# Orbiter-Finance/Plonky2-lib

Hardware: AMD Instinct MI355X
Metric: proofs/sec for secp256k1 ECDSA-verify circuit; Goldilocks NTT GB/s vs HBM peak (higher is better)
Workload: dtype u64 (Goldilocks, 64-bit modular integer)

## Files before the change

plonky2-lib_amd/csrc/merkle.hip:

```cpp
#include "merkle.h"
#include "keccak.h"
#include "poseidon.h"

namespace glp {
using namespace glf;

constexpr size_t MERKLE_COOP_MAX_PARENTS = 8192;

size_t merkle_num_digests(size_t nleaves, int cap_height) {
    size_t t = 0, w = nleaves, cap = (size_t)1 << cap_height;
    for (;;) { t += w; if (w <= cap) break; w >>= 1; }
    return t;
}
size_t merkle_cap_offset(size_t nleaves, int cap_height) {
    return merkle_num_digests(nleaves, cap_height) - ((size_t)1 << cap_height);
}

__device__ __forceinline__ void store_digest(u64 *dst, const u64 s[12]) {
    ulonglong2 a, b;
    a.x = s[0]; a.y = s[1]; b.x = s[2]; b.y = s[3];
    reinterpret_cast<ulonglong2 *>(dst)[0] = a;
    reinterpret_cast<ulonglong2 *>(dst)[1] = b;
}

__global__ __launch_bounds__(256, 4) void k_leaf_hash_lde(const u64 *__restrict__ lde, u64 *__restrict__ digests,
                                                       u32 ncols, int lg, int rate_bits, size_t lde_stride, size_t dig_stride) {
    lde += (size_t)blockIdx.y * lde_stride; digests += (size_t)blockIdx.y * dig_stride;
    const size_t N = (size_t)1 << (lg + rate_bits);
    const size_t pos = (size_t)blockIdx.x * 256 + threadIdx.x;
    if (pos >= N) return;
    const u32 r = (u32)(pos >> lg), q = (u32)(pos & (((size_t)1 << lg) - 1));
    const size_t leaf = ((size_t)bitrev32(r, rate_bits) << lg) | bitrev32(q, lg);
    u64 s[12];
#pragma unroll
    for (int i = 0; i < 12; i++) s[i] = 0;
    const u64 *p = lde + pos;
    if (ncols <= 4) {
        for (u32 c = 0; c < ncols; c++) s[c] = p[(size_t)c * N];
    } else {
        u64 nx[8];
#pragma unroll
        for (int i = 0; i < 8; i++) nx[i] = i < (int)ncols ? p[(size_t)i * N] : 0;
        for (u32 c = 0; c < ncols; c += 8) {
#pragma unroll
            for (int i = 0; i < 8; i++)
                if (c + i < ncols) s[i] = nx[i];
            if (c + 8 < ncols) {
#pragma unroll
                for (int i = 0; i < 8; i++)
                    if (c + 8 + i < ncols) nx[i] = p[(size_t)(c + 8 + i) * N];
            }
            pos::permute(s);
        }
    }
    store_digest(digests + 4 * leaf, s);
}

__global__ __launch_bounds__(256) void k_leaf_hash_lde_coop(const u64 *__restrict__ lde, u64 *__restrict__ digests,
                                                            u32 ncols, int lg, int rate_bits, size_t lde_stride, size_t dig_stride) {
    lde += (size_t)blockIdx.y * lde_stride; digests += (size_t)blockIdx.y * dig_stride;
    const size_t N = (size_t)1 << (lg + rate_bits);
    const int tid = threadIdx.x, l = tid & 15, lane = tid & 63, group_base = lane & ~15;
    const size_t pos = (size_t)blockIdx.x * 16 + (tid >> 4);
    const bool live = pos < N;
    const size_t p = live ? pos : 0;
    const u32 r = (u32)(p >> lg), q = (u32)(p & (((size_t)1 << lg) - 1));
    const size_t leaf = ((size_t)bitrev32(r, rate_bits) << lg) | bitrev32(q, lg);
    u64 x = 0;
    if (ncols <= 4) {
        if (live && l < 4) digests[4 * leaf + l] = (u32)l < ncols ? lde[(size_t)l * N + p] : 0;
        return;
    }
    for (u32 c = 0; c < ncols; c += 8) {
        if (l < 8 && c + l < ncols) x = lde[(size_t)(c + l) * N + p];
        x = pos::permute_coop(x, l, group_base);
    }
    if (live && l < 4) digests[4 * leaf + l] = x;
}

__global__ __launch_bounds__(256) void k_leaf_hash_lde_quad(const u64 *__restrict__ lde, u64 *__restrict__ digests,
                                                            u32 ncols, int lg, int rate_bits, size_t lde_stride, size_t dig_stride) {
    lde += (size_t)blockIdx.y * lde_stride; digests += (size_t)blockIdx.y * dig_stride;
    const size_t N = (size_t)1 << (lg + rate_bits);
    const int tid = threadIdx.x, q = tid & 3;
    const size_t pos = (size_t)blockIdx.x * 64 + (tid >> 2);
    const bool live = pos < N;
    const size_t p = live ? pos : 0;
    const u32 r = (u32)(p >> lg), qq = (u32)(p & (((size_t)1 << lg) - 1));
    const size_t leaf = ((size_t)bitrev32(r, rate_bits) << lg) | bitrev32(qq, lg);
    if (ncols <= 4) {
        if (live) digests[4 * leaf + q] = (u32)q < ncols ? lde[(size_t)q * N + p] : 0;
        return;
    }
    u64 x[3] = {0, 0, 0};
    for (u32 c = 0; c < ncols; c += 8) {
#pragma unroll
        for (int s = 0; s < 3; s++) {
            const u32 e = 3 * q + s;
            if (e < 8 && c + e < ncols) x[s] = lde[(size_t)(c + e) * N + p];
        }
        pos::permute_quad(x, q);
    }
    if (live) {
        if (q == 0) { digests[4 * leaf] = x[0]; digests[4 * leaf + 1] = x[1]; digests[4 * leaf + 2] = x[2]; }
        if (q == 1) digests[4 * leaf + 3] = x[0];
    }
}

__global__ __launch_bounds__(256, 4) void k_leaf_hash_rows(const u64 *__restrict__ rows, u64 *__restrict__ digests,
                                                        size_t nleaves, u32 leaf_len) {
    const size_t j = (size_t)blockIdx.x * 256 + threadIdx.x;
    if (j >= nleaves) return;
    u64 s[12];
#pragma unroll
    for (int i = 0; i < 12; i++) s[i] = 0;
    const u64 *p = rows + j * leaf_len;
    if (leaf_len <= 4) {
        for (u32 c = 0; c < leaf_len; c++) s[c] = p[c];
    } else {
        u32 c = 0;
        for (; c + 8 <= leaf_len; c += 8) {
#pragma unroll
            for (int i = 0; i < 8; i++) s[i] = p[c + i];
            pos::permute(s);
        }
        if (c < leaf_len) {
#pragma unroll
            for (int i = 0; i < 8; i++)
                if (c + i < leaf_len) s[i] = p[c + i];
            pos::permute(s);
        }
    }
    store_digest(digests + 4 * j, s);
}

__global__ __launch_bounds__(256) void k_merkle_level(const u64 *__restrict__ in, u64 *__restrict__ out, size_t m, size_t dig_stride) {
    in += (size_t)blockIdx.y * dig_stride; out += (size_t)blockIdx.y * dig_stride;
    const size_t i = (size_t)blockIdx.x * 256 + threadIdx.x;
    if (i >= m) return;
    const ulonglong2 *src = reinterpret_cast<const ulonglong2 *>(in + 8 * i);
    ulonglong2 a = src[0], b = src[1], c2 = src[2], d = src[3];
    u64 s[12] = {a.x, a.y, b.x, b.y, c2.x, c2.y, d.x, d.y, 0, 0, 0, 0};
    pos::permute(s);
    store_digest(out + 4 * i, s);
}

__global__ __launch_bounds__(256) void k_merkle_level_coop(const u64 *__restrict__ in, u64 *__restrict__ out, size_t m, size_t dig_stride) {
    in += (size_t)blockIdx.y * dig_stride; out += (size_t)blockIdx.y * dig_stride;
    const int tid = threadIdx.x, l = tid & 15, lane = tid & 63, group_base = lane & ~15;
    const size_t i = (size_t)blockIdx.x * 16 + (tid >> 4);
    const bool live = i < m;
    u64 x = (live && l < 8) ? in[8 * i + l] : 0;
    x = pos::permute_coop(x, l, group_base);
    if (live && l < 4) out[4 * i + l] = x;
}

__global__ __launch_bounds__(256) void k_merkle_level_quad(const u64 *__restrict__ in, u64 *__restrict__ out, size_t m, size_t dig_stride) {
    in += (size_t)blockIdx.y * dig_stride; out += (size_t)blockIdx.y * dig_stride;
    const int tid = threadIdx.x, q = tid & 3;
    const size_t i0 = (size_t)blockIdx.x * 64 + (tid >> 2);
    const bool live = i0 < m;
    const size_t i = live ? i0 : 0;
    u64 x[3];
#pragma unroll
    for (int s = 0; s < 3; s++) x[s] = 3 * q + s < 8 ? in[8 * i + 3 * q + s] : 0;
    pos::permute_quad(x, q);
    if (live) {
        if (q == 0) { out[4 * i] = x[0]; out[4 * i + 1] = x[1]; out[4 * i + 2] = x[2]; }
        if (q == 1) out[4 * i + 3] = x[0];
    }
}

__global__ void k_permute_states(u64 *states, size_t count) {
    const size_t i = (size_t)blockIdx.x * blockDim.x + threadIdx.x;
    if (i >= count) return;
    u64 s[12];
#pragma unroll
    for (int k = 0; k < 12; k++) s[k] = states[12 * i + k];
    pos::permute(s);
#pragma unroll
    for (int k = 0; k < 12; k++) states[12 * i + k] = s[k];
}

__global__ __launch_bounds__(256) void k_leaf_hash_lde_keccak(const u64 *__restrict__ lde, u64 *__restrict__ digests, u32 ncols, int lg,
                                                              int rate_bits, size_t lde_stride, size_t dig_stride) {
    lde += (size_t)blockIdx.y * lde_stride; digests += (size_t)blockIdx.y * dig_stride;
    const size_t N = (size_t)1 << (lg + rate_bits);
    const size_t pos = (size_t)blockIdx.x * 256 + threadIdx.x;
    if (pos >= N) return;
    const u32 r = (u32)(pos >> lg), q = (u32)(pos & (((size_t)1 << lg) - 1));
    const size_t leaf = ((size_t)bitrev32(r, rate_bits) << lg) | bitrev32(q, lg);
    const u64 *p = lde + pos;
    u64 d[4] = {0, 0, 0, 0};
    if (ncols <= 3) {
        for (u32 c = 0; c < ncols; c++) d[c] = p[(size_t)c * N];
    } else {
        kec::Sponge s;
        kec::sponge_init(s);
        u32 c = 0;
        for (; c + kec::RATE_LANES <= ncols; c += kec::RATE_LANES) {
#pragma unroll
            for (int i = 0; i < kec::RATE_LANES; i++) s.a[i] ^= p[(size_t)(c + i) * N];
            kec::f1600(s.a);
        }
#pragma unroll
        for (int i = 0; i < kec::RATE_LANES; i++) if (c + i < ncols) s.a[i] ^= p[(size_t)(c + i) * N];
        s.fill = (int)(ncols - c);
        kec::sponge_finish(s);
        kec::sponge_digest25(s, d);
    }
    store_digest(digests + 4 * leaf, d);
}
__global__ __launch_bounds__(256) void k_merkle_level_keccak(const u64 *__restrict__ in, u64 *__restrict__ out, size_t m, size_t dig_stride) {
    in += (size_t)blockIdx.y * dig_stride; out += (size_t)blockIdx.y * dig_stride;
    const size_t i = (size_t)blockIdx.x * 256 + threadIdx.x;
    if (i >= m) return;
    const ulonglong2 *src = reinterpret_cast<const ulonglong2 *>(in + 8 * i);
    const ulonglong2 a = src[0], b = src[1], c2 = src[2], e = src[3];
    const u64 l[4] = {a.x, a.y, b.x, b.y}, r[4] = {c2.x, c2.y, e.x, e.y};
    u64 d[4];
    kec::two_to_one(l, r, d);
    store_digest(out + 4 * i, d);
}

static int build_levels(glp_ctx *c, u64 *dev_digests, size_t nleaves, int cap_height, u32 K = 1, size_t dig_stride = 0, int hasher = 0) {
    size_t w = nleaves, cap = (size_t)1 << cap_height;
    u64 *lvl = dev_digests;
    while (w > cap) {
        u64 *nxt = lvl + 4 * w;
        size_t m = w >> 1;
        if (hasher == GLP_HASH_KECCAK25)
            hipLaunchKernelGGL(k_merkle_level_keccak, dim3((unsigned)((m + 255) / 256), K), dim3(256), 0, c->stream, lvl, nxt, m, dig_stride);
        else if (m * K <= MERKLE_COOP_MAX_PARENTS)
            hipLaunchKernelGGL(k_merkle_level_coop, dim3((unsigned)((m + 15) / 16), K), dim3(256), 0, c->stream, lvl, nxt, m, dig_stride);
        else if (m * K <= c->merkle_quad_max)
            hipLaunchKernelGGL(k_merkle_level_quad, dim3((unsigned)((m + 63) / 64), K), dim3(256), 0, c->stream, lvl, nxt, m, dig_stride);
        else
            hipLaunchKernelGGL(k_merkle_level, dim3((unsigned)((m + 255) / 256), K), dim3(256), 0, c->stream, lvl, nxt, m, dig_stride);
        GLP_HIP(hipGetLastError());
        lvl = nxt; w = m;
    }
    return GLP_OK;
}

int merkle_levels(glp_ctx *c, u64 *dev_digests, size_t nleaves, int cap_height, u32 K, size_t dig_stride, int hasher) {
    return build_levels(c, dev_digests, nleaves, cap_height, K, dig_stride, hasher);
}

int merkle_from_lde(glp_ctx *c, const u64 *dev_lde, u32 ncols, int lg, int rate_bits, int cap_height, u64 *dev_digests, u32 K,
                    size_t lde_stride, size_t dig_stride, int hasher) {
    const size_t N = (size_t)1 << (lg + rate_bits);
    if (cap_height < 0 || ((size_t)1 << cap_height) > N)
        return set_error(GLP_ERR_ARG, "cap_height=%d should be at most log2(leaves)=%d", cap_height, lg + rate_bits);
    GLP_REQUIRE(K >= 1 && K <= 65535, "batch of %u trees outside 1..65535", K);
    {
        StageScope st(c, "merkle_leaves", (double)N * K * (8.0 * ncols + 32.0));
        if (hasher == GLP_HASH_KECCAK25)
            hipLaunchKernelGGL(k_leaf_hash_lde_keccak, dim3((unsigned)((N + 255) / 256), K), dim3(256), 0, c->stream, dev_lde, dev_digests,
                               ncols, lg, rate_bits, lde_stride, dig_stride);
        else if (N * K <= c->merkle_coop_max)
            hipLaunchKernelGGL(k_leaf_hash_lde_coop, dim3((unsigned)((N + 15) / 16), K), dim3(256), 0, c->stream, dev_lde, dev_digests,
                               ncols, lg, rate_bits, lde_stride, dig_stride);
        else if (N * K <= c->merkle_quad_max)
            hipLaunchKernelGGL(k_leaf_hash_lde_quad, dim3((unsigned)((N + 63) / 64), K), dim3(256), 0, c->stream, dev_lde, dev_digests,
                               ncols, lg, rate_bits, lde_stride, dig_stride);
        else
            hipLaunchKernelGGL(k_leaf_hash_lde, dim3((unsigned)((N + 255) / 256), K), dim3(256), 0, c->stream, dev_lde, dev_digests,
                               ncols, lg, rate_bits, lde_stride, dig_stride);
        GLP_HIP(hipGetLastError());
    }
    StageScope st(c, "merkle_levels", (double)N * K * 32.0 * 1.5);
    return build_levels(c, dev_digests, N, cap_height, K, dig_stride, hasher);
}

int merkle_from_rows(glp_ctx *c, const u64 *dev_rows, size_t nleaves, u32 leaf_len, int cap_height, u64 *dev_digests) {
    if (cap_height < 0 || ((size_t)1 << cap_height) > nleaves)
        return set_error(GLP_ERR_ARG, "cap_height=%d should be at most log2(leaves)", cap_height);
    hipLaunchKernelGGL(k_leaf_hash_rows, dim3((unsigned)((nleaves + 255) / 256)), dim3(256), 0, c->stream, dev_rows,
                       dev_digests, nleaves, leaf_len);
    GLP_HIP(hipGetLastError());
    return build_levels(c, dev_digests, nleaves, cap_height);
}

__global__ void k_gather_lde_rows(const u64 *__restrict__ lde, u32 ncols, int lg, int rate_bits,
                                  const u64 *__restrict__ leaf_idx, u32 count, u64 *__restrict__ out, size_t out_stride,
                                  size_t lde_bstride, size_t out_bstride) {
    lde += (size_t)blockIdx.y * lde_bstride; leaf_idx += (size_t)blockIdx.y * count; out += (size_t)blockIdx.y * out_bstride;
    const size_t N = (size_t)1 << (lg + rate_bits);
    const size_t t = (size_t)blockIdx.x * blockDim.x + threadIdx.x;
    if (t >= (size_t)count * ncols) return;
    const u32 k = (u32)(t / ncols), col = (u32)(t % ncols);
    const u64 j = leaf_idx[k];
    const u32 rtop = (u32)(j >> lg), jl = (u32)(j & (((u64)1 << lg) - 1));
    const size_t pos = ((size_t)bitrev32(rtop, rate_bits) << lg) | bitrev32(jl, lg);
    out[(size_t)k * out_stride + col] = lde[(size_t)col * N + pos];
}

__global__ void k_gather_paths(const u64 *__restrict__ digests, size_t nleaves, int depth,
                               const u64 *__restrict__ leaf_idx, u32 idx_shift, u32 count, u64 *__restrict__ out, size_t out_stride,
                               size_t dig_bstride, size_t out_bstride) {
    digests += (size_t)blockIdx.y * dig_bstride; leaf_idx += (size_t)blockIdx.y * count; out += (size_t)blockIdx.y * out_bstride;
    const size_t t = (size_t)blockIdx.x * blockDim.x + threadIdx.x;
    if (t >= (size_t)count * depth * 4) return;
    const u32 e = (u32)(t & 3);
    const u32 lvl = (u32)((t >> 2) % depth), k = (u32)((t >> 2) / depth);
    size_t off = 0, w = nleaves;
    for (u32 l = 0; l < lvl; l++) { off += w; w >>= 1; }
    const size_t idx = ((leaf_idx[k] >> idx_shift) >> lvl) ^ 1;
    out[(size_t)k * out_stride + 4 * lvl + e] = digests[4 * (off + idx) + e];
}

int merkle_gather_lde_rows(glp_ctx *c, const u64 *dev_lde, u32 ncols, int lg, int rate_bits, const u64 *dev_leaf_idx,
                           u32 count, u64 *dev_out, size_t out_stride, u32 K, size_t lde_bstride, size_t out_bstride) {
    if (out_stride == 0) out_stride = ncols;
    const size_t total = (size_t)count * ncols;
    if (!total) return GLP_OK;
    hipLaunchKernelGGL(k_gather_lde_rows, dim3((unsigned)((total + 255) / 256), K), dim3(256), 0, c->stream, dev_lde, ncols, lg,
                       rate_bits, dev_leaf_idx, count, dev_out, out_stride, lde_bstride, out_bstride);
    GLP_HIP(hipGetLastError());
    return GLP_OK;
}

int merkle_gather_paths(glp_ctx *c, const u64 *dev_digests, size_t nleaves, int cap_height, const u64 *dev_leaf_idx,
                        u32 count, u64 *dev_out, size_t out_stride, u32 idx_shift, u32 K, size_t dig_bstride, size_t out_bstride) {
    int depth = 0;
    for (size_t w = nleaves; w > ((size_t)1 << cap_height); w >>= 1) depth++;
    if (out_stride == 0) out_stride = (size_t)depth * 4;
    const size_t total = (size_t)count * depth * 4;
    if (!total) return GLP_OK;
    hipLaunchKernelGGL(k_gather_paths, dim3((unsigned)((total + 255) / 256), K), dim3(256), 0, c->stream, dev_digests, nleaves,
                       depth, dev_leaf_idx, idx_shift, count, dev_out, out_stride, dig_bstride, out_bstride);
    GLP_HIP(hipGetLastError());
    return GLP_OK;
}

__global__ __launch_bounds__(256) void k_salt_lde(u64 *__restrict__ lde, u32 ncols, int lg, int rate_bits, size_t lde_stride,
                                                  u64 seed0, u64 seed1, u64 seed2, u64 seed3, u32 tag) {
    lde += (size_t)blockIdx.y * lde_stride;
    const size_t N = (size_t)1 << (lg + rate_bits);
    const size_t pos = (size_t)blockIdx.x * 256 + threadIdx.x;
    if (pos >= N) return;
    const u32 r = (u32)(pos >> lg), q = (u32)(pos & (((size_t)1 << lg) - 1));
    const u64 leaf = ((u64)bitrev32(r, rate_bits) << lg) | bitrev32(q, lg);
    u64 s[12] = {seed0, seed1, seed2, add(seed3, (u64)blockIdx.y), (u64)tag, leaf & 0xffffffffull, leaf >> 32, 0, 0, 0, 0, 0};
    pos::permute(s);
#pragma unroll
    for (int i = 0; i < 4; i++) lde[(size_t)(ncols + i) * N + pos] = s[i];
}

int merkle_fill_salts(glp_ctx *c, u64 *dev_lde, u32 ncols, int lg, int rate_bits, const u64 seed[4], u32 tag, u32 K, size_t lde_stride) {
    const size_t N = (size_t)1 << (lg + rate_bits);
    GLP_REQUIRE(K >= 1 && K <= 65535, "batch of %u trees outside 1..65535", K);
    for (int i = 0; i < 4; i++) GLP_REQUIRE(seed[i] < P, "salt seed word %d is not a canonical field element", i);
    StageScope st(c, "salt", (double)N * K * 32.0);
    hipLaunchKernelGGL(k_salt_lde, dim3((unsigned)((N + 255) / 256), K), dim3(256), 0, c->stream, dev_lde, ncols, lg, rate_bits, lde_stride,
                       seed[0], seed[1], seed[2], seed[3], tag);
    GLP_HIP(hipGetLastError());
    return GLP_OK;
}

int poseidon_permute_states(glp_ctx *c, u64 *dev_states, size_t count) {
    if (!count) return GLP_OK;
    hipLaunchKernelGGL(k_permute_states, dim3((unsigned)((count + 255) / 256)), dim3(256), 0, c->stream, dev_states, count);
    GLP_HIP(hipGetLastError());
    return GLP_OK;
}

}
```

plonky2-lib_amd/csrc/poseidon.h:

```cpp
#pragma once
#include "glf.h"
#include "poseidon_rc.inc"

namespace pos {
using namespace glf;

#if defined(__HIP_DEVICE_COMPILE__)
static __device__ const u64 RC[360] = { GLP_POSEIDON_RC_LIST };
#else
static const u64 RC[360] = { GLP_POSEIDON_RC_LIST };
#endif

GLF_HD u64 sbox7(u64 x) {
    u64 x2 = sqr(x), x4 = sqr(x2), x3 = mul(x, x2);
    return mul(x3, x4);
}

GLF_HD void mds_layer(u64 s[12]) {
    constexpr u32 C[12] = {17, 15, 41, 16, 2, 28, 13, 13, 39, 18, 34, 20};
    u32 lo[12], hi[12];
#pragma unroll
    for (int i = 0; i < 12; i++) { lo[i] = (u32)s[i]; hi[i] = (u32)(s[i] >> 32); }
#pragma unroll
    for (int r = 0; r < 12; r++) {
        u64 al = 0, ah = 0;
#pragma unroll
        for (int i = 0; i < 12; i++) {
            al += (u64)lo[(i + r) % 12] * C[i];
            ah += (u64)hi[(i + r) % 12] * C[i];
        }
        if (r == 0) { al += (u64)lo[0] * 8; ah += (u64)hi[0] * 8; }
        u64 l = al + (ah << 32);
        u32 h = (u32)(ah >> 32) + (l < al ? 1u : 0u);
        s[r] = reduce96(l, h);
    }
}

GLF_HD void permute_ref(u64 s[12]) {
    int rc = 0;
    for (int r = 0; r < 4; r++) {
#pragma unroll
        for (int i = 0; i < 12; i++) s[i] = sbox7(add(s[i], RC[rc + i]));
        rc += 12;
        mds_layer(s);
    }
    for (int r = 0; r < 22; r++) {
#pragma unroll
        for (int i = 0; i < 12; i++) s[i] = add(s[i], RC[rc + i]);
        rc += 12;
        s[0] = sbox7(s[0]);
        mds_layer(s);
    }
    for (int r = 0; r < 4; r++) {
#pragma unroll
        for (int i = 0; i < 12; i++) s[i] = sbox7(add(s[i], RC[rc + i]));
        rc += 12;
        mds_layer(s);
    }
}

GLF_HD u32 mds_entry(int r, int i) {
    constexpr u32 C[12] = {17, 15, 41, 16, 2, 28, 13, 13, 39, 18, 34, 20};
    return C[(i - r + 12) % 12] + (r == 0 && i == 0 ? 8u : 0u);
}
namespace pblk {
constexpr u64 PRIME = 0xFFFFFFFF00000001ULL;
constexpr u32 CIRC[12] = {17, 15, 41, 16, 2, 28, 13, 13, 39, 18, 34, 20};
constexpr u64 RC_CE[360] = { GLP_POSEIDON_RC_LIST };
constexpr bool pow_round0_add_fits(int i = 0) { return i == 8 || (RC_CE[i] < 0xFFFFFE0000000000ULL && pow_round0_add_fits(i + 1)); }
static_assert(pow_round0_add_fits(), "RC[0..7] must stay below 2^64 - 2^41: k_pow_batch2 adds the candidate without reduction");
constexpr u64 m_at(int r, int c) { return CIRC[(c - r + 12) % 12] + ((r == 0 && c == 0) ? 8u : 0u); }
template <int K, bool MERGED> struct Tab {
    u32 g0[K][12] = {};
    u32 gK[12][12] = {};
    u32 bt[K][12] = {};
    u64 max_weight = 0;
};
template <int K, bool MERGED> constexpr Tab<K, MERGED> make_tab() {
    Tab<K, MERGED> t{};
    u64 A[12][12] = {}, N[12][12] = {}, G[12][12] = {};
    for (int r = 0; r < 12; r++) for (int c = 0; c < 12; c++) A[r][c] = m_at(r, c);
    for (int j = 1; j <= K; j++) {
        if (j > 1) {
            for (int r = 0; r < 12; r++) for (int c = 0; c < 12; c++) {
                u64 acc = 0;
                for (int k = 1; k < 12; k++) acc += m_at(r, k) * A[k][c];
                N[r][c] = acc;
            }
            for (int r = 0; r < 12; r++) for (int c = 0; c < 12; c++) A[r][c] = N[r][c];
        }
        for (int r = 0; r < 12; r++) for (int c = 0; c < 12; c++) {
            u64 acc = 0;
            if (MERGED) { for (int k = 1; k < 12; k++) acc += A[r][k] * m_at(k, c); }
            else acc = c == 0 ? 0 : A[r][c];
            G[r][c] = acc;
        }
        if (j < K) for (int c = 0; c < 12; c++) t.g0[j - 1][c] = (u32)G[0][c];
    }
    for (int r = 0; r < 12; r++) for (int c = 0; c < 12; c++) t.gK[r][c] = (u32)G[r][c];
    for (int r = 0; r < 12; r++) t.bt[0][r] = (u32)m_at(r, 0);
    for (int s = 1; s < K; s++)
        for (int r = 0; r < 12; r++) {
            u64 acc = 0;
            for (int k = 1; k < 12; k++) acc += m_at(r, k) * t.bt[s - 1][k];
            t.bt[s][r] = (u32)acc;
        }
    for (int r = 0; r < 12; r++) {
        u64 w = 0;
        for (int c = 0; c < 12; c++) { w += G[r][c]; if (G[r][c] >> 32) w = ~0ULL >> 1; }
        for (int i = 1; i <= K; i++) w += t.bt[K - i][r];
        if (w > t.max_weight) t.max_weight = w;
    }
    return t;
}
template <int K> struct BlkConst { u64 kpre; u64 k0[K]; u64 kK[12]; };
template <int K, bool MERGED> constexpr BlkConst<K> make_blk(int first_round) {
    BlkConst<K> b{};
    u64 kc[12] = {}, nx[12] = {};
    for (int i = 0; i < 12; i++) kc[i] = RC_CE[12 * (first_round + (MERGED ? 0 : 1)) + i];
    b.kpre = MERGED ? kc[0] : 0;
    for (int j = MERGED ? 1 : 2; j <= K; j++) {
        for (int r = 0; r < 12; r++) {
            unsigned __int128 acc = RC_CE[12 * (first_round + j) + r];
            for (int k = 1; k < 12; k++) acc += (unsigned __int128)m_at(r, k) * kc[k];
            nx[r] = (u64)(acc % PRIME);
        }
        for (int r = 0; r < 12; r++) kc[r] = nx[r];
        if (j < K) b.k0[j - 1] = kc[0];
    }
    if (!MERGED && K > 1) b.k0[0] = RC_CE[12 * (first_round + 1)];
    b.k0[K - 1] = 0;
    for (int r = 0; r < 12; r++) b.kK[r] = kc[r];
    return b;
}
}

#if defined(__HIP_DEVICE_COMPILE__)
static __device__ const u64 RC_ZERO[12] = {0, 0, 0, 0, 0, 0, 0, 0, 0, 0, 0, 0};

__device__ __forceinline__ u64 sbox7_nc(u64 x) {
#ifdef GLP_SBOX_PLAIN_MUL
    const u64 x2 = mul_nc(x, x), x4 = mul_nc(x2, x2), x3 = mul_nc(x, x2);
    return mul_nc(x3, x4);
#else
    const u64 x2 = mul_nc_cc(x, x), x4 = mul_nc_cc(x2, x2), x3 = mul_nc_cc(x, x2);
    return mul_nc_cc(x3, x4);
#endif
}
#ifndef GLP_MDS_GROUP
#define GLP_MDS_GROUP 4
#endif
#ifndef GLP_SBOX_GROUP
#define GLP_SBOX_GROUP 4
#endif
__device__ __forceinline__ void sbox_layer_nc(u64 s[12]) {
#pragma unroll
    for (int i = 0; i < 12; i++) {
        s[i] = sbox7_nc(s[i]);
        if (i % GLP_SBOX_GROUP == GLP_SBOX_GROUP - 1) __builtin_amdgcn_sched_barrier(0);
    }
}
__device__ __forceinline__ void mds_add_nc(u64 s[12], const u64 *rc) {
    constexpr u32 C[12] = {17, 15, 41, 16, 2, 28, 13, 13, 39, 18, 34, 20};
    u32 lo[12], hi[12];
#pragma unroll
    for (int i = 0; i < 12; i++) { lo[i] = (u32)s[i]; hi[i] = (u32)(s[i] >> 32); }
    u32 c16 = 16, c2 = 2;
    asm volatile("" : "+s"(c16), "+s"(c2));
#pragma unroll
    for (int r = 0; r < 12; r++) {
        u64 al = (u64)(u32)rc[r] + (u64)lo[r] * (r == 0 ? C[0] + 8 : C[0]);
        asm("" : "+v"(al));
#pragma unroll
        for (int i = 1; i < 12; i++) al += (u64)lo[(i + r) % 12] * (C[i] == 16 ? c16 : C[i] == 2 ? c2 : C[i]);
        u64 ah = (al >> 32) + (rc[r] >> 32);
#pragma unroll
        for (int i = 0; i < 12; i++) ah += (u64)hi[(i + r) % 12] * (i == 0 && r == 0 ? C[0] + 8 : C[i] == 16 ? c16 : C[i] == 2 ? c2 : C[i]);
#ifdef GLP_MDS_FOLD_C
        s[r] = fold96_c((ah << 32) | (u32)al, (u32)(ah >> 32));
#else
        s[r] = fold96_nc((ah << 32) | (u32)al, (u32)(ah >> 32));
#endif
        if (r % GLP_MDS_GROUP == GLP_MDS_GROUP - 1) __builtin_amdgcn_sched_barrier(0);
    }
}

static __device__ const pblk::BlkConst<3> PBM[1] = {pblk::make_blk<3, true>(4)};
static __device__ const pblk::BlkConst<4> PB4[4] = {pblk::make_blk<4, false>(7), pblk::make_blk<4, false>(11),
                                                    pblk::make_blk<4, false>(15), pblk::make_blk<4, false>(19)};
static __device__ const pblk::BlkConst<3> PB3[1] = {pblk::make_blk<3, false>(23)};

#define GLP_PB_ROW(OUT, GROW, KCONST, NS, BCOEF)                                                    \
    do {                                                                                            \
        const u64 _k = (KCONST);                                                                    \
        u64 al = (u32)_k;                                                                           \
        _Pragma("unroll") for (int c = 0; c < 12; c++) if ((GROW)[c] != 0) al += (u64)lo[c] * (GROW)[c];   \
        _Pragma("unroll") for (int i = 0; i < (NS); i++) al += (u64)slo[i] * (BCOEF);               \
        u64 ah = (al >> 32) + (_k >> 32);                                                           \
        _Pragma("unroll") for (int c = 0; c < 12; c++) if ((GROW)[c] != 0) ah += (u64)hi[c] * (GROW)[c];   \
        _Pragma("unroll") for (int i = 0; i < (NS); i++) ah += (u64)shi[i] * (BCOEF);               \
        (OUT) = fold96_nc((ah << 32) | (u32)al, (u32)(ah >> 32));                                   \
    } while (0)

template <int K, bool MERGED, class Hook>
__device__ __forceinline__ void partial_block_nc(u64 s[12], const pblk::BlkConst<K> &kc, Hook hook) {
    constexpr pblk::Tab<K, MERGED> T = pblk::make_tab<K, MERGED>();
    static_assert(T.max_weight + 2 < (1ULL << 32), "unreduced accumulation would overflow");
    u32 lo[12], hi[12], slo[K], shi[K];
#pragma unroll
    for (int i = 0; i < 12; i++) { lo[i] = (u32)s[i]; hi[i] = (u32)(s[i] >> 32); }
    u64 x0 = s[0];
    if constexpr (MERGED) {
        constexpr u32 MROW0[12] = {25, 15, 41, 16, 2, 28, 13, 13, 39, 18, 34, 20};
        GLP_PB_ROW(x0, MROW0, kc.kpre, 0, 0u);
    }
    u64 sig = sbox7_nc(hook(0, x0));
    slo[0] = (u32)sig; shi[0] = (u32)(sig >> 32);
#pragma unroll
    for (int j = 1; j < K; j++) {
        u64 z;
        GLP_PB_ROW(z, T.g0[j - 1], kc.k0[j - 1], j, T.bt[j - 1 - i][0]);
        sig = sbox7_nc(hook(j, z));
        slo[j] = (u32)sig; shi[j] = (u32)(sig >> 32);
    }
#pragma unroll
    for (int r = 0; r < 12; r++) {
        GLP_PB_ROW(s[r], T.gK[r], kc.kK[r], K, T.bt[K - 1 - i][r]);
        if (r % GLP_MDS_GROUP == GLP_MDS_GROUP - 1) __builtin_amdgcn_sched_barrier(0);
    }
}

template <int K, bool MERGED>
__device__ __forceinline__ void partial_block_nc(u64 s[12], const pblk::BlkConst<K> &kc) {
    partial_block_nc<K, MERGED>(s, kc, [](int, u64 z) { return z; });
}

struct FullNext { u64 k[8][12]; };
constexpr FullNext make_full_next() {
    FullNext f{};
    for (int r = 0; r < 3; r++) for (int i = 0; i < 12; i++) { f.k[r][i] = pblk::RC_CE[12 * (r + 1) + i]; f.k[4 + r][i] = pblk::RC_CE[12 * (27 + r) + i]; }
    return f;
}
static __device__ const FullNext RCN = make_full_next();

__device__ __forceinline__ void permute(u64 s[12]) {
#pragma unroll
    for (int i = 0; i < 12; i++) s[i] = add(s[i], RC[i]);
#ifdef GLP_POSEIDON_PLAIN_PARTIAL
    int rc = 12;
    for (int r = 0; r < 4; r++) { sbox_layer_nc(s); mds_add_nc(s, RC + rc); rc += 12; }
    for (int r = 0; r < 22; r++) { s[0] = sbox7_nc(s[0]); mds_add_nc(s, RC + rc); rc += 12; }
    for (int r = 0; r < 3; r++) { sbox_layer_nc(s); mds_add_nc(s, RC + rc); rc += 12; }
    sbox_layer_nc(s);
    mds_add_nc(s, RC_ZERO);
#else
#ifdef GLP_POSEIDON_FLAT
#define GLP_FULL_ROUND(i) sbox_layer_nc(s); mds_add_nc(s, RCN.k[i]);
    GLP_FULL_ROUND(0) GLP_FULL_ROUND(1) GLP_FULL_ROUND(2)
    sbox_layer_nc(s);
    partial_block_nc<3, true>(s, PBM[0]);
    partial_block_nc<4, false>(s, PB4[0]); partial_block_nc<4, false>(s, PB4[1]);
    partial_block_nc<4, false>(s, PB4[2]); partial_block_nc<4, false>(s, PB4[3]);
    partial_block_nc<3, false>(s, PB3[0]);
    GLP_FULL_ROUND(4) GLP_FULL_ROUND(5) GLP_FULL_ROUND(6) GLP_FULL_ROUND(7)
#undef GLP_FULL_ROUND
#else
#pragma nounroll
    for (int half = 0; half < 2; half++) {
#pragma nounroll
        for (int r = 0; r < 4; r++) {
            sbox_layer_nc(s);
            if (half == 0 && r == 3) break;
            mds_add_nc(s, RCN.k[4 * half + r]);
        }
        if (half == 0) {
            partial_block_nc<3, true>(s, PBM[0]);
#pragma nounroll
            for (int b = 0; b < 4; b++) partial_block_nc<4, false>(s, PB4[b]);
            partial_block_nc<3, false>(s, PB3[0]);
        }
    }
#endif
#endif
#pragma unroll
    for (int i = 0; i < 12; i++) s[i] = canon(s[i]);
}
__device__ __forceinline__ void pow_round0_consts(const u64 st[12], u32 pos, u64 out[12]) {
    u64 c[12];
    for (int i = 0; i < 12; i++) c[i] = (u32)i == pos ? 0 : canon(sbox7_nc(add(st[i], RC[i])));
    for (int r = 0; r < 12; r++) {
        u64 acc = RC[12 + r];
        for (int i = 0; i < 12; i++) if ((u32)i != pos) acc = add(acc, mul(c[i], (u64)mds_entry(r, i)));
        out[r] = acc;
    }
}
template <class GiveUp>
__device__ __forceinline__ u64 permute_tail7(u64 s[12], GiveUp give_up) {
#pragma nounroll
    for (int half = 0; half < 2; half++) {
#pragma nounroll
        for (int r = half == 0 ? 1 : 0; r < 4; r++) {
            sbox_layer_nc(s);
            if (r == 3) break;
            mds_add_nc(s, RCN.k[4 * half + r]);
            if (half == 1 && r == 1 && give_up()) return ~0ull;
        }
        if (half == 0) {
            if (give_up()) return ~0ull;
            partial_block_nc<3, true>(s, PBM[0]);
#pragma nounroll
            for (int b = 0; b < 4; b++) {
                partial_block_nc<4, false>(s, PB4[b]);
                if (b == 1 && give_up()) return ~0ull;
            }
            partial_block_nc<3, false>(s, PB3[0]);
            if (give_up()) return ~0ull;
        }
    }
    constexpr u32 C[12] = {17, 15, 41, 16, 2, 28, 13, 13, 39, 18, 34, 20};
    u64 al = 0, ah = 0;
#pragma unroll
    for (int i = 0; i < 12; i++) { al += (u64)(u32)s[(i + 7) % 12] * C[i]; ah += (u64)(u32)(s[(i + 7) % 12] >> 32) * C[i]; }
    ah += al >> 32;
    return canon(fold96_nc((ah << 32) | (u32)al, (u32)(ah >> 32)));
}
__device__ __forceinline__ u64 permute_tail7(u64 s[12]) { return permute_tail7(s, [] { return false; }); }
static __device__ const u32 MDS_C24[24] = {17, 15, 41, 16, 2, 28, 13, 13, 39, 18, 34, 20, 17, 15, 41, 16, 2, 28, 13, 13, 39, 18, 34, 20};
template <int J> __device__ __forceinline__ u64 row_bcast(u64 v) {
    return (u64)__builtin_amdgcn_update_dpp((long long)0, (long long)v, 0x150 + J, 0xf, 0xf, true);
}
template <int J> __device__ __forceinline__ void coop_row_terms(u64 &al, u64 &ah, u64 x, const u32 (&cf)[12]) {
    if constexpr (J < 12) {
        const u64 b = row_bcast<J>(x);
        al += (u64)(u32)b * cf[J];
        ah += (u64)(u32)(b >> 32) * cf[J];
        coop_row_terms<J + 1>(al, ah, x, cf);
    }
}
__device__ __forceinline__ u64 permute_coop(u64 x, int l , int ) {
    const int ll = l < 12 ? l : 0;
    u32 cf[12];
#pragma unroll
    for (int j = 0; j < 12; j++) cf[j] = MDS_C24[12 + j - ll];
    if (l == 0) cf[0] += 8;
    x = add(x, RC[ll]);
    for (int r = 0; r < 30; r++) {
        const bool full = r < 4 || r >= 26;
        const u64 sb = sbox7_nc(x);
        if (full || l == 0) x = sb;
        const u64 rcn = r < 29 ? RC[12 * (r + 1) + ll] : 0;
        u64 al = (u32)rcn, ah = rcn >> 32;
        coop_row_terms<0>(al, ah, x, cf);
        ah += al >> 32;
        x = fold96_nc((ah << 32) | (u32)al, (u32)(ah >> 32));
    }
    return canon(x);
}
template <int D> __device__ __forceinline__ u32 quad_rot(u32 v) {
    constexpr int CTRL = (D & 3) | (((D + 1) & 3) << 2) | (((D + 2) & 3) << 4) | (((D + 3) & 3) << 6);
    return (u32)__builtin_amdgcn_mov_dpp((int)v, CTRL, 0xf, 0xf, true);
}
__device__ __forceinline__ void permute_quad(u64 x[3], int q ) {
    constexpr u32 C[12] = {17, 15, 41, 16, 2, 28, 13, 13, 39, 18, 34, 20};
    const u64 *rc = RC + 3 * q;
    const u32 diag = q == 0 ? 8u : 0u;
#pragma unroll
    for (int s = 0; s < 3; s++) x[s] = add(x[s], rc[s]);
#pragma nounroll
    for (int r = 0; r < 30; r++) {
        const bool full = r < 4 || r >= 26;
        const u64 sb = sbox7_nc(x[0]);
        if (full) { x[0] = sb; x[1] = sbox7_nc(x[1]); x[2] = sbox7_nc(x[2]); }
        else if (q == 0) x[0] = sb;
        u32 lo[4][3], hi[4][3];
#pragma unroll
        for (int s = 0; s < 3; s++) {
            lo[0][s] = (u32)x[s]; hi[0][s] = (u32)(x[s] >> 32);
            lo[1][s] = quad_rot<1>(lo[0][s]); hi[1][s] = quad_rot<1>(hi[0][s]);
            lo[2][s] = quad_rot<2>(lo[0][s]); hi[2][s] = quad_rot<2>(hi[0][s]);
            lo[3][s] = quad_rot<3>(lo[0][s]); hi[3][s] = quad_rot<3>(hi[0][s]);
        }
#pragma unroll
        for (int a = 0; a < 3; a++) {
            const u64 rcn = r < 29 ? rc[12 * (r + 1) + a] : 0;
            u64 al = (u32)rcn;
#pragma unroll
            for (int i = 0; i < 12; i++) al += (u64)lo[((a + i) / 3) & 3][(a + i) % 3] * C[i];
            if (a == 0) al += (u64)lo[0][0] * diag;
            u64 ah = (al >> 32) + (rcn >> 32);
#pragma unroll
            for (int i = 0; i < 12; i++) ah += (u64)hi[((a + i) / 3) & 3][(a + i) % 3] * C[i];
            if (a == 0) ah += (u64)hi[0][0] * diag;
            x[a] = fold96_nc((ah << 32) | (u32)al, (u32)(ah >> 32));
        }
    }
#pragma unroll
    for (int s = 0; s < 3; s++) x[s] = canon(x[s]);
}
__device__ __forceinline__ u64 shfl64(u64 v, int src) {
    const u32 lo = (u32)__shfl((int)(u32)v, src, 64), hi = (u32)__shfl((int)(u32)(v >> 32), src, 64);
    return ((u64)hi << 32) | lo;
}
__device__ __forceinline__ u64 shfl_xor64(u64 v, int m) {
    const u32 lo = (u32)__shfl_xor((int)(u32)v, m, 64), hi = (u32)__shfl_xor((int)(u32)(v >> 32), m, 64);
    return ((u64)hi << 32) | lo;
}
#else
namespace host {
inline u64 sbox(u64 x) { return sbox7(x); }
inline u64 fold(u64 al, u64 ah, u64 k) {
    al += (u32)k;
    const u64 h = ah + (al >> 32) + (k >> 32);
    const u64 l = (h << 32) | (u32)al, t1 = (h >> 32) * EPS;
    u64 t2 = l + t1;
    if (t2 < t1) t2 += EPS;
    return t2;
}
inline void mds_add(u64 s[12], const u64 *rc) {
    mds_layer(s);
    for (int i = 0; i < 12; i++) s[i] = add(s[i], rc[i]);
}
template <int K, bool MERGED>
inline void partial_block(u64 s[12], const pblk::BlkConst<K> &kc) {
    constexpr pblk::Tab<K, MERGED> T = pblk::make_tab<K, MERGED>();
    static_assert(T.max_weight + 2 < (1ULL << 32), "unreduced accumulation would overflow");
    u32 lo[12], hi[12], slo[K], shi[K];
    for (int i = 0; i < 12; i++) { lo[i] = (u32)s[i]; hi[i] = (u32)(s[i] >> 32); }
    u64 x0 = s[0];
    if (MERGED) {
        constexpr u32 MROW0[12] = {25, 15, 41, 16, 2, 28, 13, 13, 39, 18, 34, 20};
        u64 al = 0, ah = 0;
        _Pragma("unroll") for (int c = 0; c < 12; c++) { al += (u64)lo[c] * MROW0[c]; ah += (u64)hi[c] * MROW0[c]; }
        x0 = fold(al, ah, kc.kpre);
    }
    u64 sig = sbox(x0);
    slo[0] = (u32)sig; shi[0] = (u32)(sig >> 32);
    _Pragma("unroll") for (int j = 1; j < K; j++) {
        u64 al = 0, ah = 0;
        _Pragma("unroll") for (int c = 0; c < 12; c++) { al += (u64)lo[c] * T.g0[j - 1][c]; ah += (u64)hi[c] * T.g0[j - 1][c]; }
        _Pragma("unroll") for (int i = 0; i < j; i++) { al += (u64)slo[i] * T.bt[j - 1 - i][0]; ah += (u64)shi[i] * T.bt[j - 1 - i][0]; }
        sig = sbox(fold(al, ah, kc.k0[j - 1]));
        slo[j] = (u32)sig; shi[j] = (u32)(sig >> 32);
    }
    _Pragma("unroll") for (int r = 0; r < 12; r++) {
        u64 al = 0, ah = 0;
        _Pragma("unroll") for (int c = 0; c < 12; c++) { al += (u64)lo[c] * T.gK[r][c]; ah += (u64)hi[c] * T.gK[r][c]; }
        _Pragma("unroll") for (int i = 0; i < K; i++) { al += (u64)slo[i] * T.bt[K - 1 - i][r]; ah += (u64)shi[i] * T.bt[K - 1 - i][r]; }
        s[r] = fold(al, ah, kc.kK[r]);
    }
}
static constexpr pblk::BlkConst<3> HPBM = pblk::make_blk<3, true>(4);
static constexpr pblk::BlkConst<4> HPB4[4] = {pblk::make_blk<4, false>(7), pblk::make_blk<4, false>(11), pblk::make_blk<4, false>(15), pblk::make_blk<4, false>(19)};
static constexpr pblk::BlkConst<3> HPB3 = pblk::make_blk<3, false>(23);
}
inline void permute(u64 s[12]) {
    static const u64 ZERO12[12] = {0, 0, 0, 0, 0, 0, 0, 0, 0, 0, 0, 0};
    for (int i = 0; i < 12; i++) s[i] = add(s[i], RC[i]);
    for (int r = 0; r < 4; r++) {
        for (int i = 0; i < 12; i++) s[i] = host::sbox(s[i]);
        if (r < 3) host::mds_add(s, RC + 12 * (r + 1));
    }
    host::partial_block<3, true>(s, host::HPBM);
    for (int b = 0; b < 4; b++) host::partial_block<4, false>(s, host::HPB4[b]);
    host::partial_block<3, false>(s, host::HPB3);
    for (int r = 26; r < 30; r++) {
        for (int i = 0; i < 12; i++) s[i] = host::sbox(s[i]);
        host::mds_add(s, r < 29 ? RC + 12 * (r + 1) : ZERO12);
    }
    for (int i = 0; i < 12; i++) s[i] = canon(canon(s[i]));
}
inline u64 permute_coop(u64 x, int, int) { return x; }
inline void permute_quad(u64 *, int) {}
GLF_HD u64 sbox7_nc(u64 x) { return x; }
GLF_HD void pow_round0_consts(const u64 *, u32, u64 *) {}
GLF_HD u64 permute_tail7(u64 *) { return 0; }
template <class GiveUp> GLF_HD u64 permute_tail7(u64 *, GiveUp) { return 0; }
GLF_HD u64 shfl64(u64 v, int) { return v; }
GLF_HD u64 shfl_xor64(u64 v, int) { return v; }
#endif

GLF_HD void two_to_one(const u64 l[4], const u64 r[4], u64 out[4]) {
    u64 s[12];
#pragma unroll
    for (int i = 0; i < 4; i++) { s[i] = l[i]; s[4 + i] = r[i]; s[8 + i] = 0; }
    permute(s);
#pragma unroll
    for (int i = 0; i < 4; i++) out[i] = s[i];
}

}
```

profiles/isa_slots.py:

```python
#!/usr/bin/env python3
import collections
import json
import os
import re
import subprocess
import sys
import tempfile

ROOT = os.path.dirname(os.path.dirname(os.path.abspath(__file__)))
HALF_WEIGHT = 1.75
FULL = {"v_add_u32_e32", "v_sub_u32_e32", "v_subrev_u32_e32", "v_xor_b32_e32", "v_and_b32_e32", "v_or_b32_e32", "v_mov_b32_e32",
        "v_lshrrev_b32_e32", "v_not_b32_e32", "v_cndmask_b32_e32", "v_accvgpr_write_b32", "v_accvgpr_read_b32"}


def main():
    src = os.path.join(ROOT, "plonky2-lib_amd", "csrc", "merkle.hip")
    with tempfile.TemporaryDirectory() as td:
        out = os.path.join(td, "merkle.s")
        subprocess.check_call(["/opt/rocm/bin/hipcc", "--offload-arch=gfx950", "-O3", "-std=c++17", "-DGLP_LDE_NO_HOIST", "-DGLP_POSEIDON_FLAT", "-S", "--cuda-device-only",
                               "-o", out, src], stderr=subprocess.DEVNULL)
        txt = open(out).read()
    body = txt[txt.index("_ZN3glp16k_permute_statesEPmm:"):]
    body = body[:body.index("s_endpgm")]
    ops = []
    labels = set()
    for l in body.split("\n"):
        m = re.match(r"^(\.LBB\d+_\d+):", l)
        if m:
            labels.add(m.group(1))
            continue
        m = re.match(r"^\s+([vs]_\w+|ds_\w+|global_\w+)(.*)", l)
        if m:
            if m.group(1).startswith("s_cbranch") and any(lab in m.group(2) for lab in labels):
                raise SystemExit("backward branch in the flat build: loops were not fully unrolled")
            ops.append(m.group(1))
    c = collections.Counter(ops)
    valu = sum(v for k, v in c.items() if k.startswith("v_"))
    slots = sum(v * (1.0 if k in FULL else HALF_WEIGHT) for k, v in c.items() if k.startswith("v_"))
    out = {"build": "-DGLP_POSEIDON_FLAT (all round loops unrolled; the shipped build keeps them rolled: same instructions per round)",
           "mads_per_permutation": c["v_mad_u64_u32"], "valu_instructions": valu, "s_nop": c["s_nop"],
           "full_rate_instructions": sum(v for k, v in c.items() if k in FULL),
           "slots_per_permutation": slots, "top_opcodes": dict(c.most_common(14))}
    json.dump(out, sys.stdout, indent=1)
    print()


if __name__ == "__main__":
    main()
```

Measured before the change: 9.114.

## Compute Poseidon full-round MDS layer with int8 MFMA across the wavefront

```diff
diff --git a/plonky2-lib_amd/csrc/merkle.hip b/plonky2-lib_amd/csrc/merkle.hip
--- a/plonky2-lib_amd/csrc/merkle.hip
+++ b/plonky2-lib_amd/csrc/merkle.hip
@@ -27,10 +27,12 @@
                                                        u32 ncols, int lg, int rate_bits, size_t lde_stride, size_t dig_stride) {
     lde += (size_t)blockIdx.y * lde_stride; digests += (size_t)blockIdx.y * dig_stride;
     const size_t N = (size_t)1 << (lg + rate_bits);
-    const size_t pos = (size_t)blockIdx.x * 256 + threadIdx.x;
-    if (pos >= N) return;
+    const size_t pos0 = (size_t)blockIdx.x * 256 + threadIdx.x;
+    const bool live = pos0 < N;
+    const size_t pos = live ? pos0 : 0;
     const u32 r = (u32)(pos >> lg), q = (u32)(pos & (((size_t)1 << lg) - 1));
     const size_t leaf = ((size_t)bitrev32(r, rate_bits) << lg) | bitrev32(q, lg);
+    const pos::MdsOperands mo = pos::mds_operands();
     u64 s[12];
 #pragma unroll
     for (int i = 0; i < 12; i++) s[i] = 0;
@@ -50,10 +52,10 @@
                 for (int i = 0; i < 8; i++)
                     if (c + 8 + i < ncols) nx[i] = p[(size_t)(c + 8 + i) * N];
             }
-            pos::permute(s);
-        }
-    }
-    store_digest(digests + 4 * leaf, s);
+            pos::permute_wave(s, mo);
+        }
+    }
+    if (live) store_digest(digests + 4 * leaf, s);
 }
 
 __global__ __launch_bounds__(256) void k_leaf_hash_lde_coop(const u64 *__restrict__ lde, u64 *__restrict__ digests,
@@ -109,8 +111,10 @@
 
 __global__ __launch_bounds__(256, 4) void k_leaf_hash_rows(const u64 *__restrict__ rows, u64 *__restrict__ digests,
                                                         size_t nleaves, u32 leaf_len) {
-    const size_t j = (size_t)blockIdx.x * 256 + threadIdx.x;
-    if (j >= nleaves) return;
+    const size_t j0 = (size_t)blockIdx.x * 256 + threadIdx.x;
+    const bool live = j0 < nleaves;
+    const size_t j = live ? j0 : 0;
+    const pos::MdsOperands mo = pos::mds_operands();
     u64 s[12];
 #pragma unroll
     for (int i = 0; i < 12; i++) s[i] = 0;
@@ -122,27 +126,29 @@
         for (; c + 8 <= leaf_len; c += 8) {
 #pragma unroll
             for (int i = 0; i < 8; i++) s[i] = p[c + i];
-            pos::permute(s);
+            pos::permute_wave(s, mo);
         }
         if (c < leaf_len) {
 #pragma unroll
             for (int i = 0; i < 8; i++)
                 if (c + i < leaf_len) s[i] = p[c + i];
-            pos::permute(s);
-        }
-    }
-    store_digest(digests + 4 * j, s);
+            pos::permute_wave(s, mo);
+        }
+    }
+    if (live) store_digest(digests + 4 * j, s);
 }
 
 __global__ __launch_bounds__(256) void k_merkle_level(const u64 *__restrict__ in, u64 *__restrict__ out, size_t m, size_t dig_stride) {
     in += (size_t)blockIdx.y * dig_stride; out += (size_t)blockIdx.y * dig_stride;
-    const size_t i = (size_t)blockIdx.x * 256 + threadIdx.x;
-    if (i >= m) return;
+    const size_t i0 = (size_t)blockIdx.x * 256 + threadIdx.x;
+    const bool live = i0 < m;
+    const size_t i = live ? i0 : 0;
+    const pos::MdsOperands mo = pos::mds_operands();
     const ulonglong2 *src = reinterpret_cast<const ulonglong2 *>(in + 8 * i);
     ulonglong2 a = src[0], b = src[1], c2 = src[2], d = src[3];
     u64 s[12] = {a.x, a.y, b.x, b.y, c2.x, c2.y, d.x, d.y, 0, 0, 0, 0};
-    pos::permute(s);
-    store_digest(out + 4 * i, s);
+    pos::permute_wave(s, mo);
+    if (live) store_digest(out + 4 * i, s);
 }
 
 __global__ __launch_bounds__(256) void k_merkle_level_coop(const u64 *__restrict__ in, u64 *__restrict__ out, size_t m, size_t dig_stride) {
@@ -172,14 +178,18 @@
 }
 
 __global__ void k_permute_states(u64 *states, size_t count) {
-    const size_t i = (size_t)blockIdx.x * blockDim.x + threadIdx.x;
-    if (i >= count) return;
+    const size_t i0 = (size_t)blockIdx.x * blockDim.x + threadIdx.x;
+    const bool live = i0 < count;
+    const size_t i = live ? i0 : 0;
+    const pos::MdsOperands mo = pos::mds_operands();
     u64 s[12];
 #pragma unroll
     for (int k = 0; k < 12; k++) s[k] = states[12 * i + k];
-    pos::permute(s);
-#pragma unroll
-    for (int k = 0; k < 12; k++) states[12 * i + k] = s[k];
+    pos::permute_wave(s, mo);
+    if (live) {
+#pragma unroll
+        for (int k = 0; k < 12; k++) states[12 * i + k] = s[k];
+    }
 }
 
 __global__ __launch_bounds__(256) void k_leaf_hash_lde_keccak(const u64 *__restrict__ lde, u64 *__restrict__ digests, u32 ncols, int lg,
diff --git a/plonky2-lib_amd/csrc/poseidon.h b/plonky2-lib_amd/csrc/poseidon.h
--- a/plonky2-lib_amd/csrc/poseidon.h
+++ b/plonky2-lib_amd/csrc/poseidon.h
@@ -185,6 +185,82 @@
     }
 }
 
+static __device__ const u32 MDS_C24[24] = {17, 15, 41, 16, 2, 28, 13, 13, 39, 18, 34, 20, 17, 15, 41, 16, 2, 28, 13, 13, 39, 18, 34, 20};
+typedef int v4i32 __attribute__((ext_vector_type(4)));
+typedef int v16i32 __attribute__((ext_vector_type(16)));
+struct MdsOperands { v4i32 a[3]; };
+__device__ __forceinline__ MdsOperands mds_operands() {
+    const u32 lane = __builtin_amdgcn_mbcnt_hi(~0u, __builtin_amdgcn_mbcnt_lo(~0u, 0u));
+    const u32 row = lane & 31, h = lane >> 5, rl = row >> 3, b = row & 3;
+    const bool mine = ((row >> 2) & 1) == h;
+    MdsOperands mo;
+#pragma unroll
+    for (int d = 0; d < 3; d++)
+#pragma unroll
+        for (int e = 0; e < 4; e++) mo.a[d][e] = mine ? (int)(MDS_C24[12 + 4 * d + e - rl] << (8 * b)) : 0;
+    return mo;
+}
+__device__ __forceinline__ long long mad_i64_i32_one(int a, long long k) {
+    long long o;
+    asm("v_mad_i64_i32 %0, vcc, %1, 1, %2" : "=&v"(o) : "v"(a), "s"(k) : "vcc");
+    return o;
+}
+__device__ __forceinline__ long long mad_i64_i32_one_v(int a, long long k) {
+    long long o;
+    asm("v_mad_i64_i32 %0, vcc, %1, 1, %2" : "=&v"(o) : "v"(a), "v"(k) : "vcc");
+    return o;
+}
+__device__ __forceinline__ long long mad_i64_i32(int a, int b_uniform, long long c) {
+    long long o;
+    asm("v_mad_i64_i32 %0, vcc, %1, %2, %3" : "=&v"(o) : "v"(a), "s"(b_uniform), "v"(c) : "vcc");
+    return o;
+}
+#define GLP_MDS_WAVE_ROW(D, RL, KTERM) \
+    mad_i64_i32((D)[4 * (RL) + 2] + ((D)[4 * (RL) + 3] << 8), c64k, KTERM)
+__device__ __forceinline__ void mds_add_wave(u64 s[12], const u64 *rc, const MdsOperands &mo) {
+    v4i32 bl[3], bh[3];
+#pragma unroll
+    for (int q = 0; q < 3; q++)
+#pragma unroll
+        for (int e = 0; e < 4; e++) {
+            bl[q][e] = (int)((u32)s[4 * q + e] ^ 0x80808080u);
+            bh[q][e] = (int)((u32)(s[4 * q + e] >> 32) ^ 0x80808080u);
+        }
+    const u32 lo0 = (u32)s[0], hi0 = (u32)(s[0] >> 32);
+    int c64k = 65536;
+    asm volatile("" : "+s"(c64k));
+    constexpr u64 BIAS = (u64)(128u * 256u) * 0x01010101ull;
+#pragma unroll
+    for (int g = 0; g < 3; g++) {
+        long long al[4];
+        {
+            v16i32 d = {0, 0, 0, 0, 0, 0, 0, 0, 0, 0, 0, 0, 0, 0, 0, 0};
+#pragma unroll
+            for (int q = 0; q < 3; q++) d = __builtin_amdgcn_mfma_i32_32x32x32_i8(mo.a[(q - g + 3) % 3], bl[q], d, 0, 0, 0);
+#pragma unroll
+            for (int rl = 0; rl < 4; rl++) {
+                const int r = 4 * g + rl, x = d[4 * rl] + (d[4 * rl + 1] << 8);
+                const u64 k = BIAS + (u32)rc[r];
+                al[rl] = GLP_MDS_WAVE_ROW(d, rl, r == 0 ? mad_i64_i32_one_v(x, (long long)((u64)lo0 * 8u + k)) : mad_i64_i32_one(x, (long long)k));
+            }
+        }
+        {
+            v16i32 d = {0, 0, 0, 0, 0, 0, 0, 0, 0, 0, 0, 0, 0, 0, 0, 0};
+#pragma unroll
+            for (int q = 0; q < 3; q++) d = __builtin_amdgcn_mfma_i32_32x32x32_i8(mo.a[(q - g + 3) % 3], bh[q], d, 0, 0, 0);
+#pragma unroll
+            for (int rl = 0; rl < 4; rl++) {
+                const int r = 4 * g + rl, x = d[4 * rl] + (d[4 * rl + 1] << 8) + (int)(al[rl] >> 32);
+                const u64 k = BIAS + (rc[r] >> 32);
+                const long long ah = GLP_MDS_WAVE_ROW(d, rl, r == 0 ? mad_i64_i32_one_v(x, (long long)((u64)hi0 * 8u + k)) : mad_i64_i32_one(x, (long long)k));
+                s[r] = fold96_nc(((u64)ah << 32) | (u32)al[rl], (u32)((u64)ah >> 32));
+            }
+        }
+        __builtin_amdgcn_sched_barrier(0);
+    }
+}
+#undef GLP_MDS_WAVE_ROW
+
 static __device__ const pblk::BlkConst<3> PBM[1] = {pblk::make_blk<3, true>(4)};
 static __device__ const pblk::BlkConst<4> PB4[4] = {pblk::make_blk<4, false>(7), pblk::make_blk<4, false>(11),
                                                     pblk::make_blk<4, false>(15), pblk::make_blk<4, false>(19)};
@@ -243,19 +319,29 @@
 }
 static __device__ const FullNext RCN = make_full_next();
 
-__device__ __forceinline__ void permute(u64 s[12]) {
+template <bool WAVE>
+__device__ __forceinline__ void permute_body(u64 s[12], const MdsOperands &mo) {
+#if defined(GLP_POSEIDON_VALU_MDS)
+    constexpr bool MATRIX = false;
+#else
+    constexpr bool MATRIX = WAVE;
+#endif
+    auto full_mds = [&](const u64 *rcp) __attribute__((always_inline)) {
+        if constexpr (MATRIX) mds_add_wave(s, rcp, mo);
+        else mds_add_nc(s, rcp);
+    };
 #pragma unroll
     for (int i = 0; i < 12; i++) s[i] = add(s[i], RC[i]);
 #ifdef GLP_POSEIDON_PLAIN_PARTIAL
     int rc = 12;
-    for (int r = 0; r < 4; r++) { sbox_layer_nc(s); mds_add_nc(s, RC + rc); rc += 12; }
+    for (int r = 0; r < 4; r++) { sbox_layer_nc(s); full_mds(RC + rc); rc += 12; }
     for (int r = 0; r < 22; r++) { s[0] = sbox7_nc(s[0]); mds_add_nc(s, RC + rc); rc += 12; }
-    for (int r = 0; r < 3; r++) { sbox_layer_nc(s); mds_add_nc(s, RC + rc); rc += 12; }
+    for (int r = 0; r < 3; r++) { sbox_layer_nc(s); full_mds(RC + rc); rc += 12; }
     sbox_layer_nc(s);
-    mds_add_nc(s, RC_ZERO);
+    full_mds(RC_ZERO);
 #else
 #ifdef GLP_POSEIDON_FLAT
-#define GLP_FULL_ROUND(i) sbox_layer_nc(s); mds_add_nc(s, RCN.k[i]);
+#define GLP_FULL_ROUND(i) sbox_layer_nc(s); full_mds(RCN.k[i]);
     GLP_FULL_ROUND(0) GLP_FULL_ROUND(1) GLP_FULL_ROUND(2)
     sbox_layer_nc(s);
     partial_block_nc<3, true>(s, PBM[0]);
@@ -271,7 +357,7 @@
         for (int r = 0; r < 4; r++) {
             sbox_layer_nc(s);
             if (half == 0 && r == 3) break;
-            mds_add_nc(s, RCN.k[4 * half + r]);
+            full_mds(RCN.k[4 * half + r]);
         }
         if (half == 0) {
             partial_block_nc<3, true>(s, PBM[0]);
@@ -285,6 +371,8 @@
 #pragma unroll
     for (int i = 0; i < 12; i++) s[i] = canon(s[i]);
 }
+__device__ __forceinline__ void permute(u64 s[12]) { permute_body<false>(s, MdsOperands{}); }
+__device__ __forceinline__ void permute_wave(u64 s[12], const MdsOperands &mo) { permute_body<true>(s, mo); }
 __device__ __forceinline__ void pow_round0_consts(const u64 st[12], u32 pos, u64 out[12]) {
     u64 c[12];
     for (int i = 0; i < 12; i++) c[i] = (u32)i == pos ? 0 : canon(sbox7_nc(add(st[i], RC[i])));
@@ -325,7 +413,6 @@
     return canon(fold96_nc((ah << 32) | (u32)al, (u32)(ah >> 32)));
 }
 __device__ __forceinline__ u64 permute_tail7(u64 s[12]) { return permute_tail7(s, [] { return false; }); }
-static __device__ const u32 MDS_C24[24] = {17, 15, 41, 16, 2, 28, 13, 13, 39, 18, 34, 20, 17, 15, 41, 16, 2, 28, 13, 13, 39, 18, 34, 20};
 template <int J> __device__ __forceinline__ u64 row_bcast(u64 v) {
     return (u64)__builtin_amdgcn_update_dpp((long long)0, (long long)v, 0x150 + J, 0xf, 0xf, true);
 }
@@ -469,6 +556,9 @@
     }
     for (int i = 0; i < 12; i++) s[i] = canon(canon(s[i]));
 }
+struct MdsOperands { int unused; };
+inline MdsOperands mds_operands() { return MdsOperands{}; }
+inline void permute_wave(u64 s[12], const MdsOperands &) { permute(s); }
 inline u64 permute_coop(u64 x, int, int) { return x; }
 inline void permute_quad(u64 *, int) {}
 GLF_HD u64 sbox7_nc(u64 x) { return x; }
diff --git a/profiles/isa_slots.py b/profiles/isa_slots.py
--- a/profiles/isa_slots.py
+++ b/profiles/isa_slots.py
@@ -9,6 +9,7 @@
 
 ROOT = os.path.dirname(os.path.dirname(os.path.abspath(__file__)))
 HALF_WEIGHT = 1.75
+MFMA_SLOTS = 16
 FULL = {"v_add_u32_e32", "v_sub_u32_e32", "v_subrev_u32_e32", "v_xor_b32_e32", "v_and_b32_e32", "v_or_b32_e32", "v_mov_b32_e32",
         "v_lshrrev_b32_e32", "v_not_b32_e32", "v_cndmask_b32_e32", "v_accvgpr_write_b32", "v_accvgpr_read_b32"}
 
@@ -31,16 +32,18 @@
             continue
         m = re.match(r"^\s+([vs]_\w+|ds_\w+|global_\w+)(.*)", l)
         if m:
-            if m.group(1).startswith("s_cbranch") and any(lab in m.group(2) for lab in labels):
+            if m.group(1).startswith("s_cbranch") and m.group(2).strip() in labels:
                 raise SystemExit("backward branch in the flat build: loops were not fully unrolled")
             ops.append(m.group(1))
     c = collections.Counter(ops)
-    valu = sum(v for k, v in c.items() if k.startswith("v_"))
-    slots = sum(v * (1.0 if k in FULL else HALF_WEIGHT) for k, v in c.items() if k.startswith("v_"))
+    mfma = sum(v for k, v in c.items() if k.startswith("v_mfma"))
+    valu = sum(v for k, v in c.items() if k.startswith("v_") and not k.startswith("v_mfma"))
+    slots = sum(v * (1.0 if k in FULL else HALF_WEIGHT) for k, v in c.items() if k.startswith("v_") and not k.startswith("v_mfma"))
     out = {"build": "-DGLP_POSEIDON_FLAT (all round loops unrolled; the shipped build keeps them rolled: same instructions per round)",
            "mads_per_permutation": c["v_mad_u64_u32"], "valu_instructions": valu, "s_nop": c["s_nop"],
            "full_rate_instructions": sum(v for k, v in c.items() if k in FULL),
-           "slots_per_permutation": slots, "top_opcodes": dict(c.most_common(14))}
+           "slots_per_permutation": slots, "mfma_instructions": mfma, "matrix_pipe_slots": MFMA_SLOTS * mfma,
+           "slots_with_matrix_pipe": slots + MFMA_SLOTS * mfma, "top_opcodes": dict(c.most_common(14))}
     json.dump(out, sys.stdout, indent=1)
     print()
 
```

New measurement: 9.243, median of 6. 1.01x the previous value.
